# janinethoma/soft_contrastive_learning

Measured on AMD Instinct MI355X. Metric: train-step images/sec (VGG16-NetVLAD soft-MS, 640x480), higher is better.
Workload: dtype bf16; 1 GPU; configs[1]: wms soft-contrastive train step, VGG16-NetVLAD K=64, 24 images/GPU 640x480, bf16 backbone, float32-accurate NetVLAD + f32 loss; global_batch=24, locations=1200, parallelism=dp1, optimizer=adam

## Files before the change

soft_contrastive_learning_amd/csrc/convh.hip:

```cpp
#include <mutex>

#include "conv_lds.h"
#include "conv_pack_layout.h"

namespace {

constexpr int HBW = 40;
constexpr int HWC = HBW + 2;
constexpr int HPIX = 32;
constexpr int HCCH = 32;
constexpr int HNB = 128;
constexpr int HTPB = 3;
constexpr int HWT = 4 * HNB * 8;
constexpr int HTHR = 512;
constexpr int HX = 1;

template <int BHv>
struct HCfg {
  static constexpr int BH = BHv == 24 ? 12 : BHv;
  static constexpr int WR = BH + 2;
  static constexpr int SLOTS = WR * HWC * 4;
  static constexpr int NI = (SLOTS + 511) / 512;
  static constexpr int NA = (NI + 1) / 2;
  static constexpr int WIN = NI * 8 * 512;
  static constexpr int NMT = BH / 2 * 5;
  static constexpr int MT = BHv == 24 ? 15 : BH == 12 ? 8 : BH == 8 ? 10 : 4;
  static constexpr int NT = (BHv == 24 || BH == 8) ? 2 : 4;
  static constexpr int SPT = BHv == 24 ? 3 : 2;
  static constexpr int MH = MT / SPT;
  static constexpr size_t LDS = (2 * (size_t)WIN + 3 * HTPB * (size_t)HWT) * 2;
};

template <int V>
struct HConst {
  static constexpr int value = V;
};

__device__ __forceinline__ int ht_row(int i) { return (i >= 4 && i < 12) ? 1 : 0; }
__device__ __forceinline__ int ht_col(int i) { return i < 4 ? i : i < 8 ? i - 4 : i < 12 ? i - 4 : i - 8; }

__global__ __launch_bounds__(256) void convh_pack_kernel(const void* __restrict__ w, int64_t sk,
                                                         int64_t sc, int64_t sh, int64_t sw,
                                                         int flags, int cin, int kout,
                                                         unsigned short* __restrict__ packed) {
  const int transposed = flags & 1, wf32 = flags & 2;
  const int64_t idx = (int64_t)blockIdx.x * 256 + threadIdx.x;
  const int64_t total = (int64_t)9 * (cin / HCCH) * kout * HCCH;
  if (idx >= total) return;
  const int64_t off = pack_src_offset(pack_lds_coord(idx, cin), sk, sc, sh, sw, transposed);
  packed[idx] = weight_bf16(w, off, wf32);
}

template <int EPI, int BHv, bool STAMP = false, bool FULL = false>
__global__ __launch_bounds__(HTHR, 1) void convh_kernel(const unsigned short* __restrict__ x,
                                                       const unsigned short* __restrict__ packed,
                                                       int B, int H, int W, int cin, int kout,
                                                       unsigned short* __restrict__ out,
                                                       const float* __restrict__ bias, int relu,
                                                       const unsigned short* __restrict__ mask,
                                                       unsigned char* __restrict__ pidx,
                                                       int vblocks) {
  using G = HCfg<BHv>;
  constexpr int BH = G::BH, WR = G::WR, WIN = G::WIN, NMT = G::NMT, MT = G::MT, NT = G::NT;
  constexpr int MH = G::MH, NI = G::NI, NA = G::NA, SPT = G::SPT;
  constexpr bool WEAVE = BHv == 24 || BHv == 6 || BHv == 8;
  constexpr int HS = 9 * SPT;
  extern __shared__ __attribute__((aligned(16))) unsigned short lds[];
  unsigned short* win = lds;
  unsigned short* wts = lds + 2 * WIN;
  const int lane = threadIdx.x & 63;
  const int wid = __builtin_amdgcn_readfirstlane(threadIdx.x >> 6);
  const int i = lane & 15, g = lane >> 4;
  const int kb = kout / HNB;
  const int blocks_x = (W + HBW - 1) / HBW, blocks_y = (H + BH - 1) / BH;
  const int CC = cin / HCCH, S = 9 * CC;
  const unsigned short* zeros = reinterpret_cast<const unsigned short*>(zero_block);
  int nb = 0, b = 0, y0 = 0, x0 = 0;
  int rel[NI];
#pragma unroll
  for (int n = 0; n < NI; ++n) {
    const int slot = 64 * (wid + 8 * n) + lane;
    const int pix = slot >> 2, row = pix / HWC, col = pix - row * HWC;
    const int piece = (slot & 3) ^ (((col >> 2) & 1) | ((row & 1) << 1));
    rel[n] = pix >= WR * HWC ? -1 : (row << 16) | (col << 8) | piece;
  }
  int woff[NI];
  auto locate = [&](int vb) -> bool {
    const int grp = vb / (8 * kb), rem = vb - grp * 8 * kb;
    const int pblk = grp * 8 + (rem & 7);
    nb = rem >> 3;
    if (pblk >= B * blocks_x * blocks_y) return false;
    b = pblk / (blocks_x * blocks_y);
    const int t2 = pblk % (blocks_x * blocks_y);
    y0 = (t2 / blocks_x) * BH;
    x0 = (t2 % blocks_x) * HBW;
#pragma unroll
    for (int n = 0; n < NI; ++n) {
      int r = rel[n];
      asm volatile("" : "+v"(r));
      const int y = y0 - 1 + (r >> 16), xx = x0 - 1 + ((r >> 8) & 255);
      const bool inimg = r >= 0 && y >= 0 && y < H && xx >= 0 && xx < W;
      woff[n] = inimg ? ((b * H + y) * W + xx) * cin + 8 * (r & 255) : -1;
    }
    return true;
  };
  auto issue_win = [&](int cc, int buf, int n0, int n1) {
    const unsigned base = lds_byte_of(win) + buf * WIN * 2;
#pragma unroll
    for (int n = 0; n < NI; ++n)
      if (n >= n0 && n < n1)
        glds16(woff[n] >= 0 ? x + woff[n] + HCCH * cc : zeros, base + (wid + 8 * n) * 1024);
  };
  auto issue_wts = [&](int grp, int buf) {
    const unsigned short* src = packed + ((int64_t)nb * S + HTPB * grp) * HWT + lane * 8;
    const unsigned base = lds_byte_of(wts) + buf * HTPB * HWT * 2;
#pragma unroll
    for (int n = 0; n < 3; ++n) {
      const int j = wid + 8 * n;
      glds16(src + j * 512, base + j * 1024);
    }
  };
  auto issue_wts_one = [&](int grp, int buf, int n) {
    const unsigned short* src = packed + ((int64_t)nb * S + HTPB * grp) * HWT + lane * 8;
    const unsigned base = lds_byte_of(wts) + buf * HTPB * HWT * 2;
    const int j = wid + 8 * n;
    glds16(src + j * 512, base + j * 1024);
  };
  auto stage_first = [&]() {
    issue_wts(0, 0);
    issue_wts(1, 1);
    issue_win(0, 0, 0, NI);
  };
  const int mg = NT == 4 ? wid >> 1 : wid >> 2, ng = NT == 4 ? wid & 1 : wid & 3;
  constexpr bool REG = MT % 5 == 0;
  constexpr bool ALLT = NMT % MT == 0;
  int aoff[MT];
#pragma unroll
  for (int j = 0; j < MT; ++j) {
    const int mt = MT * mg + j < NMT ? MT * mg + j : NMT - 1;
    aoff[j] = ((2 * (mt / 5)) * HWC + 8 * (mt % 5)) * HPIX;
  }
  const int lane_a = (ht_row(i) * HWC + ht_col(i)) * HPIX + (REG ? 2 * (MT / 5) * mg * HWC * HPIX : 0);
  int pieces = 0;
#pragma unroll
  for (int t = 0; t < 9; ++t) {
    const int r = ht_row(i) + t / 3, c = ht_col(i) + t % 3;
    pieces |= (g ^ (((c >> 2) & 1) | ((r & 1) << 1))) << (2 * t);
  }
  const int lane_b = (g * HNB + 16 * NT * ng + i) * 8;

  const int relu_in = relu;
  const int dbg = STAMP ? 0 : SCL_DIAG_ONLY(relu >> 1);
  relu &= 1;
  const short relu_floor = relu ? (short)0 : (short)-32768;
  bool staged = false;
  if (!STAMP && (dbg & 4) && wid >= 4) __builtin_amdgcn_s_setprio(1);
  uint64_t stamp[STAMP ? 24 : 1];
  int tcount = 0;
#define HSTAMP(k)                                                                     \
  if (STAMP)                                                                          \
  asm volatile("s_memtime %0\n\ts_waitcnt lgkmcnt(0)" : "=s"(stamp[STAMP ? (k) : 0])::"memory")
  for (int vb = blockIdx.x; vb < vblocks; vb += gridDim.x) {
    HSTAMP(0);
    if (!staged) {
      if (!locate(vb)) continue;
      stage_first();
    }
    staged = false;
    const int nb_t = nb, b_t = b, y0_t = y0, x0_t = x0;

    f32x4 acc[MT][NT];
#pragma unroll
    for (int j = 0; j < MT; ++j)
#pragma unroll
      for (int n = 0; n < NT; ++n) acc[j][n] = f32x4{0.f, 0.f, 0.f, 0.f};

    u32x4 af[2][MH], bf[2][NT];
    int tb = 0;
    auto load_half = [&](const unsigned short* wbase, int h, int par, int apar) {
      const int t = h / SPT, mh = h % SPT;
      if (mh == 0) {
        const unsigned short* wbp = wts + t * HWT + lane_b;
#pragma unroll
        for (int n = 0; n < NT; ++n)
          bf[(t + par) & 1][n] = *reinterpret_cast<const u32x4*>(wbp + 16 * n * 8);
        int pk = pieces;
        asm volatile("" : "+v"(pk));
        tb = lane_a + ((pk >> (2 * t)) & 3) * 8;
      }
#pragma unroll
      for (int j = 0; j < MH; ++j)
        af[(h + apar) & 1][j] = *reinterpret_cast<const u32x4*>(
            wbase + tb +
            (REG ? (2 * ((MH * mh + j) / 5) * HWC + 8 * ((MH * mh + j) % 5)) * HPIX : aoff[MH * mh + j]) +
            ((t / 3) * HWC + t % 3) * HPIX);
    };
    const int NG = 3 * CC;
    auto chunk = [&](int cc, auto par_c) {
      constexpr int PAR = decltype(par_c)::value;
      constexpr int APAR = PAR * (HS & 1);
      const unsigned short* wcur = win + (cc & 1) * WIN;
      const unsigned short* wnext = win + ((cc + 1) & 1) * WIN;
      const int ccn = cc + 1 < CC ? cc + 1 : cc;
      auto issue_op = [&](int gi, int k) {
        if (k < 3) {
          const int gn = 3 * cc + gi + 2 < NG ? 3 * cc + gi + 2 : NG - 3 + (gi + 2) % 3;
          issue_wts_one(gn, (gi + 2) % 3, k);
        } else {
          const int n = (gi == 0 ? 0 : NA) + k - 3;
          if (gi == 0 && n < NA) issue_win(ccn, (cc + 1) & 1, n, n + 1);
          if (gi == 1 && n < NI) issue_win(ccn, (cc + 1) & 1, n, n + 1);
        }
      };
#pragma unroll
      for (int h = 0; h < HS; ++h) {
        if (h + 1 < HS)
          load_half(wcur, h + 1, PAR, APAR);
        else
          load_half(wnext, 0, PAR ^ 1, APAR ^ (HS & 1));
        __builtin_amdgcn_sched_barrier(0);
        const int t = h / SPT, mh = h % SPT;
        const bool after_barrier = WEAVE && (h % (3 * SPT) == HX + 1);
#pragma unroll
        for (int j = 0; j < MH; ++j) {
#pragma unroll
          for (int n = 0; n < NT; ++n)
            acc[MH * mh + j][n] =
                EPI == 3 ? mfma16b(af[(h + APAR) & 1][j], bf[(t + PAR) & 1][n], acc[MH * mh + j][n])
                         : mfma16b(bf[(t + PAR) & 1][n], af[(h + APAR) & 1][j], acc[MH * mh + j][n]);
          if (after_barrier) {
            __builtin_amdgcn_sched_barrier(0);
#pragma unroll
            for (int k = j * 6 / MH; k < (j + 1) * 6 / MH; ++k) issue_op(h / (3 * SPT), k);
            __builtin_amdgcn_sched_barrier(0);
          }
        }
        if (h % (3 * SPT) == HX) {
          __builtin_amdgcn_sched_barrier(0);
          const int gi = h / (3 * SPT);
          if (gi == 1)
            asm volatile("s_waitcnt vmcnt(%0)" ::"n"(NA) : "memory");
          else
            asm volatile("s_waitcnt vmcnt(0)" ::: "memory");
          HSTAMP(2 + 9 * PAR + 3 * gi);
          __builtin_amdgcn_s_barrier();
          HSTAMP(2 + 9 * PAR + 3 * gi + 1);
          if (!WEAVE) {
            const int gn = 3 * cc + gi + 2 < NG ? 3 * cc + gi + 2 : NG - 3 + (gi + 2) % 3;
            issue_wts(gn, (gi + 2) % 3);
            if (gi == 0) issue_win(ccn, (cc + 1) & 1, 0, NA);
            if (gi == 1) issue_win(ccn, (cc + 1) & 1, NA, NI);
          }
          HSTAMP(2 + 9 * PAR + 3 * gi + 2);
        }
      }
    };

    if (!(dbg & 1)) {
      asm volatile("s_waitcnt vmcnt(0)" ::: "memory");
      __syncthreads();
    }
    HSTAMP(1);
    load_half(win, 0, 0, 0);
#pragma unroll 1
    for (int cc = 0; cc < CC; cc += 2) {
      chunk(cc, HConst<0>());
      chunk(cc + 1, HConst<1>());
    }

    int nb_e = nb_t, b_e = b_t, y0_e = y0_t, x0_e = x0_t;
    asm volatile("" : "+s"(nb_e), "+s"(b_e), "+s"(y0_e), "+s"(x0_e));
    HSTAMP(20);
    __builtin_amdgcn_s_barrier();
    HSTAMP(21);
    constexpr int SLD = 16 * NT + 8;
    constexpr int PCS = 2 * NT;
    constexpr int RR = 16 * PCS / 64;
    constexpr int SCRW = 16 * SLD + 8 * (16 * NT + 16);
    static_assert(4 * SCRW <= WIN && 4 * SCRW <= HTPB * HWT, "epilogue scratch must fit");
    unsigned short* scr = wid < 4 ? lds + WIN + wid * SCRW : wts + 2 * HTPB * HWT + (wid - 4) * SCRW;
    const int ch_w = HNB * nb_e + 16 * NT * ng;
    f32x4 bias4[EPI == 1 ? NT : 1];
    float bias1[EPI == 3 ? NT : 1];
    if (EPI == 1) {
#pragma unroll
      for (int n = 0; n < NT; ++n)
        bias4[n] = *reinterpret_cast<const f32x4*>(bias + ch_w + 16 * n + 4 * g);
    }
    if (EPI == 3) {
#pragma unroll
      for (int n = 0; n < NT; ++n) bias1[n] = bias[ch_w + 16 * n + i];
    }
    int piece_o[RR], piece_px[RR];
#pragma unroll
    for (int rr = 0; rr < RR; ++rr) {
      const int pp = lane + 64 * rr;
      piece_px[rr] = pp / PCS;
      piece_o[rr] = (ht_row(pp / PCS) * W + ht_col(pp / PCS)) * kout + 8 * (pp % PCS);
    }
    constexpr int PD = MT / 2;
    u32x4 mk[EPI == 2 ? MT : 1][EPI == 2 ? RR : 1];
    const int64_t tile_off = (((int64_t)b_e * H + y0_e) * W + x0_e) * kout + ch_w;
    const bool full_tile = FULL ? !(dbg & 2) : (y0_e + BH <= H && x0_e + HBW <= W && !(dbg & 2));
    auto load_mask = [&](int j) {
      const int mt = MT * mg + j;
      const int oy = y0_e + 2 * (mt / 5), ox = x0_e + 8 * (mt % 5);
      const unsigned short* mb = mask + tile_off + ((2 * (mt / 5)) * W + 8 * (mt % 5)) * kout;
#pragma unroll
      for (int rr = 0; rr < RR; ++rr) {
        if (FULL ? (ALLT || mt < NMT) : (full_tile && mt < NMT)) {
          mk[EPI == 2 ? j : 0][EPI == 2 ? rr : 0] = *reinterpret_cast<const u32x4*>(mb + piece_o[rr]);
        } else if (FULL) {
          mk[EPI == 2 ? j : 0][EPI == 2 ? rr : 0] = u32x4{0u, 0u, 0u, 0u};
        } else {
          const bool inside = mt < NMT && oy + ht_row(piece_px[rr]) < H && ox + ht_col(piece_px[rr]) < W;
          mk[EPI == 2 ? j : 0][EPI == 2 ? rr : 0] =
              inside ? *reinterpret_cast<const u32x4*>(mb + piece_o[rr]) : u32x4{0u, 0u, 0u, 0u};
        }
      }
    };
    if (EPI == 2) {
#pragma unroll
      for (int j = 0; j < PD; ++j) load_mask(j);
    }

    auto stage_next = [&]() {
      const int vn = vb + gridDim.x;
      if (vn < vblocks && locate(vn)) {
        asm volatile("s_waitcnt vmcnt(0)" ::: "memory");
        stage_first();
        staged = true;
      }
    };
    if (EPI != 2) stage_next();

    if (EPI == 3) {
      const int PH = H / 2, PW = W / 2;
      const bool upper = g == 0 || g == 3;
      const int cb = g < 2 ? 0 : 4;
      unsigned char* scr8 = reinterpret_cast<unsigned char*>(scr + 16 * SLD);
      constexpr int SLD8 = 16 * NT + 16;
#pragma unroll
      for (int jb = 0; jb < MT; jb += 4) {
#pragma unroll
        for (int jj = 0; jj < 4; ++jj) {
          const int j = jb + jj < MT ? jb + jj : MT - 1;
#pragma unroll
          for (int n = 0; n < NT; ++n) {
#pragma unroll
            for (int q0 = 0; q0 < 4; q0 += 2) {
              const float v0 = acc[j][n][q0], v1 = acc[j][n][q0 + 1];
              const float lm = fmaxf(v0, v1);
              const int li = v0 >= v1 ? 0 : 1;
              const float om = __shfl_xor(lm, 16);
              const int oi = __shfl_xor(li, 16);
              const float mu = upper ? lm : om, ml = upper ? om : lm;
              const int iu = upper ? li : oi, il = upper ? oi : li;
              const float m = fmaxf(mu, ml);
              const int k = mu >= ml ? iu : 2 + il;
              const int pl = 4 * jj + ((cb + q0) >> 1);
              if (upper) {
                scr[pl * SLD + 16 * n + i] = f32_to_bf16(fmaxf(m + bias1[n], 0.f));
                scr8[pl * SLD8 + 16 * n + i] = (unsigned char)k;
              }
            }
          }
        }
        __builtin_amdgcn_wave_barrier();
#pragma unroll
        for (int rr = 0; rr < RR; ++rr) {
          const int pp = lane + 64 * rr, pl = pp / PCS, pc = pp % PCS;
          const int mt = MT * mg + jb + (pl >> 2);
          const int py = (y0_e >> 1) + mt / 5, px = (x0_e >> 1) + 4 * (mt % 5) + (pl & 3);
          const u32x4 v = *reinterpret_cast<const u32x4*>(scr + pl * SLD + 8 * pc);
          if (jb + (pl >> 2) < MT && (FULL ? (ALLT || mt < NMT) : (mt < NMT && py < PH && px < PW && !(dbg & 2))))
            *reinterpret_cast<u32x4*>(out + (((int64_t)b_e * PH + py) * PW + px) * kout + ch_w + 8 * pc) = v;
        }
        if (lane < 16 * NT) {
          const int pl = lane / NT, pc = lane % NT;
          const int mt = MT * mg + jb + (pl >> 2);
          const int py = (y0_e >> 1) + mt / 5, px = (x0_e >> 1) + 4 * (mt % 5) + (pl & 3);
          const u32x4 v = *reinterpret_cast<const u32x4*>(scr8 + pl * SLD8 + 16 * pc);
          if (jb + (pl >> 2) < MT && (FULL ? (ALLT || mt < NMT) : (mt < NMT && py < PH && px < PW && !(dbg & 2))))
            *reinterpret_cast<u32x4*>(pidx + (((int64_t)b_e * PH + py) * PW + px) * kout + ch_w + 16 * pc) = v;
        }
        __builtin_amdgcn_wave_barrier();
      }
    } else {
      unsigned short* out_tile = out + tile_off;
#pragma unroll
      for (int j = 0; j < MT; ++j) {
        const int mt = MT * mg + j;
        if (ALLT || mt < NMT) {
          const int oy = y0_e + 2 * (mt / 5), ox = x0_e + 8 * (mt % 5);
          unsigned short* ob = out_tile + ((2 * (mt / 5)) * W + 8 * (mt % 5)) * kout;
#pragma unroll
          for (int n = 0; n < NT; ++n) {
            f32x4 v = acc[j][n];
            if (EPI == 1) v += bias4[n];
            unsigned p0 = pack2_bf16(v[0], v[1]), p1 = pack2_bf16(v[2], v[3]);
            if (EPI == 1) {
              p0 = max2_i16(p0, relu_floor);
              p1 = max2_i16(p1, relu_floor);
            }
            const u32x2 pk = {p0, p1};
            *reinterpret_cast<u32x2*>(scr + i * SLD + 16 * n + 4 * g) = pk;
          }
          __builtin_amdgcn_wave_barrier();
#pragma unroll
          for (int rr = 0; rr < RR; ++rr) {
            u32x4 v = *reinterpret_cast<const u32x4*>(scr + piece_px[rr] * SLD + 8 * ((lane + 64 * rr) % PCS));
            if (EPI == 2) v = relu_mask(v, mk[EPI == 2 ? j : 0][EPI == 2 ? rr : 0]);
            if (full_tile) {
              *reinterpret_cast<u32x4*>(ob + piece_o[rr]) = v;
            } else if (!FULL) {
              const bool inside = oy + ht_row(piece_px[rr]) < H && ox + ht_col(piece_px[rr]) < W && !(dbg & 2);
              if (inside) *reinterpret_cast<u32x4*>(ob + piece_o[rr]) = v;
            }
          }
          __builtin_amdgcn_wave_barrier();
        }
        if (EPI == 2) {
          __builtin_amdgcn_sched_barrier(0);
          if (j + PD < MT) load_mask(j + PD);
          if (j + PD == MT - 1) stage_next();
          __builtin_amdgcn_sched_barrier(0);
        }
      }
    }
    if (STAMP) {
      HSTAMP(22);
      if (threadIdx.x == 64 * ((relu_in >> 4) & 7) && (tcount == 1 || tcount == 2)) {
        uint64_t* o = reinterpret_cast<uint64_t*>(out + (int64_t)B * H * W * kout) +
                      (int64_t)(blockIdx.x * 2 + tcount - 1) * 24;
#pragma unroll
        for (int k = 0; k < 23; ++k) o[k] = stamp[STAMP ? k : 0];
      }
      ++tcount;
    }
  }
#undef HSTAMP
}

}

struct HGeom {
  const unsigned short* packed;
  int bh;
  LdsConvGrid grid;
};

template <int E, int BHV, bool STAMP = false, bool FULL = false>
static void convh_run(const LdsConvCall& c, const HGeom& g, int relu) {
  if constexpr (!STAMP && !FULL)
    if (c.H % HCfg<BHV>::BH == 0 && c.W % HBW == 0) return convh_run<E, BHV, false, true>(c, g, relu);
  static SclDeviceOnce once;
  scl_call_once(once, [] {
    (void)hipFuncSetAttribute(reinterpret_cast<const void*>(&convh_kernel<E, BHV, STAMP, FULL>),
                              hipFuncAttributeMaxDynamicSharedMemorySize, (int)HCfg<BHV>::LDS);
  });
  SCL_LAUNCH("convh_kernel", (convh_kernel<E, BHV, STAMP, FULL>), dim3(g.grid.gsize), dim3(HTHR),
             HCfg<BHV>::LDS, c.stream, (const unsigned short*)c.x, g.packed, c.B, c.H, c.W, c.cin,
             c.kout, (unsigned short*)c.out, c.bias, relu, (const unsigned short*)c.mask,
             (unsigned char*)c.pidx, g.grid.vblocks);
}
template <int BHV>
static void convh_epilogue(const LdsConvCall& c, const HGeom& g, int dbgbits) {
  if (c.pidx) convh_run<3, BHV>(c, g, dbgbits);
  else if (c.mask) convh_run<2, BHV>(c, g, dbgbits);
  else if (c.bias) convh_run<1, BHV>(c, g, (c.relu ? 1 : 0) | dbgbits);
  else convh_run<0, BHV>(c, g, 0);
}

#ifdef SCL_DIAG
static bool convh_diag(const LdsConvCall& c, const HGeom& g, int* rc);
#endif

int convh_launch(const LdsConvCall& c) {
  const int dv = SCL_DIAG_ONLY(c.dv);
  HGeom g;
  g.packed = (const unsigned short*)c.workspace;
  if (c.flags & SCL_W_PACKED) {
    g.packed = (const unsigned short*)c.w;
  } else {
    const int64_t total = (int64_t)9 * (c.cin / HCCH) * c.kout * HCCH;
    SCL_LAUNCH("convh_pack_kernel", convh_pack_kernel, dim3((unsigned)((total + 255) / 256)),
               dim3(256), 0, c.stream, c.w, c.sk, c.sc, c.sh, c.sw, c.flags, c.cin, c.kout,
               (unsigned short*)c.workspace);
  }
  const int bx = (c.W + HBW - 1) / HBW, kb = c.kout / HNB;
  const int cus = scl_conv_cus();
  g.bh = 12;
  int64_t best = -1;
  for (int cand : {12, 8, 6}) {
    const int64_t wg = (int64_t)c.B * ((c.H + cand - 1) / cand) * bx * kb;
    const int64_t cost = ((wg + cus - 1) / cus) * (cand + 2);
    if (best < 0 || cost < best) {
      best = cost;
      g.bh = cand;
    }
  }
  if (dv == 3012 || dv == 3008 || dv == 3006) g.bh = dv - 3000;
  if (dv == 3013) g.bh = 12;
  g.grid = lds_conv_grid((int64_t)c.B * ((c.H + g.bh - 1) / g.bh) * bx, kb, cus, dv);
#ifdef SCL_DIAG
  {
    int rc;
    if (convh_diag(c, g, &rc)) return rc;
  }
#endif
  const int dbgbits = (dv >= 3020 && dv < 3024) ? (dv - 3020) << 1 : (dv == 3040 ? 4 << 1 : 0);
  if (g.bh == 12) convh_epilogue<24>(c, g, dbgbits);
  else if (g.bh == 8) convh_epilogue<8>(c, g, dbgbits);
  else convh_epilogue<6>(c, g, dbgbits);
  return scl_launch_status();
}
```

soft_contrastive_learning_amd/csrc/convh_diag.hip:

```cpp
#include "convh.hip"

static bool convh_diag(const LdsConvCall& c, const HGeom& g, int* rc) {
  const int dv = c.dv;
  const bool stamps = dv >= 3024 && dv < 3040 && c.bias && !c.mask && !c.pidx && g.bh == 12;
  if (dv != 3012 && !stamps) return false;
  if (dv == 3012)
    convh_epilogue<12>(c, g, 0);
  else if (dv < 3032)
    convh_run<1, 24, true>(c, g, (c.relu ? 1 : 0) | ((dv - 3024) << 4));
  else
    convh_run<1, 12, true>(c, g, (c.relu ? 1 : 0) | ((dv - 3032) << 4));
  *rc = scl_launch_status();
  return true;
}
```

Measured before the change: 2054 images/sec.

## Prefetch next tile's input window and weights during last K-chunk of conv

In the persistent 3x3 conv kernel, the next tile's input window and first weight groups are now prefetched while the final channel chunks of the current tile are still computing, wrapping the weight-group index and window chunk around. Previously the kernel drained the pipeline and staged the next tile synchronously in the epilogue. This removes the per-tile pipeline bubble between tiles. In exchange the tile locate logic and the index arithmetic get more complex, the epilogue lane indexing is hidden from the compiler, and the old path is kept behind a diagnostic flag.

```diff
diff --git a/soft_contrastive_learning_amd/csrc/convh.hip b/soft_contrastive_learning_amd/csrc/convh.hip
--- a/soft_contrastive_learning_amd/csrc/convh.hip
+++ b/soft_contrastive_learning_amd/csrc/convh.hip
@@ -85,15 +85,16 @@
     rel[n] = pix >= WR * HWC ? -1 : (row << 16) | (col << 8) | piece;
   }
   int woff[NI];
-  auto locate = [&](int vb) -> bool {
+  auto locate = [&](int vb, bool offsets = true) -> bool {
     const int grp = vb / (8 * kb), rem = vb - grp * 8 * kb;
     const int pblk = grp * 8 + (rem & 7);
     nb = rem >> 3;
-    if (pblk >= B * blocks_x * blocks_y) return false;
     b = pblk / (blocks_x * blocks_y);
     const int t2 = pblk % (blocks_x * blocks_y);
     y0 = (t2 / blocks_x) * BH;
     x0 = (t2 % blocks_x) * HBW;
+    if (pblk >= B * blocks_x * blocks_y) return false;
+    if (!offsets) return true;
 #pragma unroll
     for (int n = 0; n < NI; ++n) {
       int r = rel[n];
@@ -150,7 +151,8 @@
   const int lane_b = (g * HNB + 16 * NT * ng + i) * 8;
 
   const int relu_in = relu;
-  const int dbg = STAMP ? 0 : SCL_DIAG_ONLY(relu >> 1);
+  const int dbg = STAMP ? 0 : SCL_DIAG_ONLY((relu >> 1) & 7);
+  const bool oldb = SCL_DIAG_ONLY(((relu >> (STAMP ? 7 : 4)) & 1) != 0);
   relu &= 1;
   const short relu_floor = relu ? (short)0 : (short)-32768;
   bool staged = false;
@@ -165,6 +167,8 @@
     if (!staged) {
       if (!locate(vb)) continue;
       stage_first();
+    } else {
+      locate(vb, false);
     }
     staged = false;
     const int nb_t = nb, b_t = b, y0_t = y0, x0_t = x0;
@@ -196,16 +200,20 @@
             ((t / 3) * HWC + t % 3) * HPIX);
     };
     const int NG = 3 * CC;
+    bool pref = false;
     auto chunk = [&](int cc, auto par_c) {
       constexpr int PAR = decltype(par_c)::value;
       constexpr int APAR = PAR * (HS & 1);
       const unsigned short* wcur = win + (cc & 1) * WIN;
       const unsigned short* wnext = win + ((cc + 1) & 1) * WIN;
-      const int ccn = cc + 1 < CC ? cc + 1 : cc;
+      const int ccn = cc + 1 < CC ? cc + 1 : pref ? 0 : cc;
+      auto next_group = [&](int gi) {
+        const int gw = 3 * cc + gi + 2;
+        return gw < NG ? gw : oldb ? NG - 3 + (gi + 2) % 3 : gw - NG;
+      };
       auto issue_op = [&](int gi, int k) {
         if (k < 3) {
-          const int gn = 3 * cc + gi + 2 < NG ? 3 * cc + gi + 2 : NG - 3 + (gi + 2) % 3;
-          issue_wts_one(gn, (gi + 2) % 3, k);
+          issue_wts_one(next_group(gi), (gi + 2) % 3, k);
         } else {
           const int n = (gi == 0 ? 0 : NA) + k - 3;
           if (gi == 0 && n < NA) issue_win(ccn, (cc + 1) & 1, n, n + 1);
@@ -246,8 +254,7 @@
           __builtin_amdgcn_s_barrier();
           HSTAMP(2 + 9 * PAR + 3 * gi + 1);
           if (!WEAVE) {
-            const int gn = 3 * cc + gi + 2 < NG ? 3 * cc + gi + 2 : NG - 3 + (gi + 2) % 3;
-            issue_wts(gn, (gi + 2) % 3);
+            issue_wts(next_group(gi), (gi + 2) % 3);
             if (gi == 0) issue_win(ccn, (cc + 1) & 1, 0, NA);
             if (gi == 1) issue_win(ccn, (cc + 1) & 1, NA, NI);
           }
@@ -265,8 +272,13 @@
 #pragma unroll 1
     for (int cc = 0; cc < CC; cc += 2) {
       chunk(cc, HConst<0>());
+      if (cc + 2 >= CC && !oldb) {
+        const int vn = vb + gridDim.x;
+        if (vn < vblocks && locate(vn)) pref = true;
+      }
       chunk(cc + 1, HConst<1>());
     }
+    staged = pref;
 
     int nb_e = nb_t, b_e = b_t, y0_e = y0_t, x0_e = x0_t;
     asm volatile("" : "+s"(nb_e), "+s"(b_e), "+s"(y0_e), "+s"(x0_e));
@@ -326,7 +338,7 @@
 
     auto stage_next = [&]() {
       const int vn = vb + gridDim.x;
-      if (vn < vblocks && locate(vn)) {
+      if (oldb && vn < vblocks && locate(vn)) {
         asm volatile("s_waitcnt vmcnt(0)" ::: "memory");
         stage_first();
         staged = true;
@@ -336,8 +348,11 @@
 
     if (EPI == 3) {
       const int PH = H / 2, PW = W / 2;
-      const bool upper = g == 0 || g == 3;
-      const int cb = g < 2 ? 0 : 4;
+      int le = lane;
+      asm volatile("" : "+v"(le));
+      const int ie = le & 15, ge = le >> 4;
+      const bool upper = ge == 0 || ge == 3;
+      const int cb = ge < 2 ? 0 : 4;
       unsigned char* scr8 = reinterpret_cast<unsigned char*>(scr + 16 * SLD);
       constexpr int SLD8 = 16 * NT + 16;
 #pragma unroll
@@ -360,8 +375,8 @@
               const int k = mu >= ml ? iu : 2 + il;
               const int pl = 4 * jj + ((cb + q0) >> 1);
               if (upper) {
-                scr[pl * SLD + 16 * n + i] = f32_to_bf16(fmaxf(m + bias1[n], 0.f));
-                scr8[pl * SLD8 + 16 * n + i] = (unsigned char)k;
+                scr[pl * SLD + 16 * n + ie] = f32_to_bf16(fmaxf(m + bias1[n], 0.f));
+                scr8[pl * SLD8 + 16 * n + ie] = (unsigned char)k;
               }
             }
           }
@@ -369,15 +384,15 @@
         __builtin_amdgcn_wave_barrier();
 #pragma unroll
         for (int rr = 0; rr < RR; ++rr) {
-          const int pp = lane + 64 * rr, pl = pp / PCS, pc = pp % PCS;
+          const int pp = le + 64 * rr, pl = pp / PCS, pc = pp % PCS;
           const int mt = MT * mg + jb + (pl >> 2);
           const int py = (y0_e >> 1) + mt / 5, px = (x0_e >> 1) + 4 * (mt % 5) + (pl & 3);
           const u32x4 v = *reinterpret_cast<const u32x4*>(scr + pl * SLD + 8 * pc);
           if (jb + (pl >> 2) < MT && (FULL ? (ALLT || mt < NMT) : (mt < NMT && py < PH && px < PW && !(dbg & 2))))
             *reinterpret_cast<u32x4*>(out + (((int64_t)b_e * PH + py) * PW + px) * kout + ch_w + 8 * pc) = v;
         }
-        if (lane < 16 * NT) {
-          const int pl = lane / NT, pc = lane % NT;
+        if (le < 16 * NT) {
+          const int pl = le / NT, pc = le % NT;
           const int mt = MT * mg + jb + (pl >> 2);
           const int py = (y0_e >> 1) + mt / 5, px = (x0_e >> 1) + 4 * (mt % 5) + (pl & 3);
           const u32x4 v = *reinterpret_cast<const u32x4*>(scr8 + pl * SLD8 + 16 * pc);
@@ -469,7 +484,7 @@
   if (c.pidx) convh_run<3, BHV>(c, g, dbgbits);
   else if (c.mask) convh_run<2, BHV>(c, g, dbgbits);
   else if (c.bias) convh_run<1, BHV>(c, g, (c.relu ? 1 : 0) | dbgbits);
-  else convh_run<0, BHV>(c, g, 0);
+  else convh_run<0, BHV>(c, g, dbgbits & 16);
 }
 
 #ifdef SCL_DIAG
@@ -509,7 +524,7 @@
     if (convh_diag(c, g, &rc)) return rc;
   }
 #endif
-  const int dbgbits = (dv >= 3020 && dv < 3024) ? (dv - 3020) << 1 : (dv == 3040 ? 4 << 1 : 0);
+  const int dbgbits = (dv >= 3020 && dv < 3024) ? (dv - 3020) << 1 : dv == 3040 ? 4 << 1 : dv == 3041 ? 16 : 0;
   if (g.bh == 12) convh_epilogue<24>(c, g, dbgbits);
   else if (g.bh == 8) convh_epilogue<8>(c, g, dbgbits);
   else convh_epilogue<6>(c, g, dbgbits);
diff --git a/soft_contrastive_learning_amd/csrc/convh_diag.hip b/soft_contrastive_learning_amd/csrc/convh_diag.hip
--- a/soft_contrastive_learning_amd/csrc/convh_diag.hip
+++ b/soft_contrastive_learning_amd/csrc/convh_diag.hip
@@ -2,12 +2,14 @@
 
 static bool convh_diag(const LdsConvCall& c, const HGeom& g, int* rc) {
   const int dv = c.dv;
-  const bool stamps = dv >= 3024 && dv < 3040 && c.bias && !c.mask && !c.pidx && g.bh == 12;
+  const bool stamps = ((dv >= 3024 && dv < 3040) || (dv >= 3042 && dv < 3050)) && c.bias && !c.mask && !c.pidx && g.bh == 12;
   if (dv != 3012 && !stamps) return false;
   if (dv == 3012)
     convh_epilogue<12>(c, g, 0);
   else if (dv < 3032)
     convh_run<1, 24, true>(c, g, (c.relu ? 1 : 0) | ((dv - 3024) << 4));
+  else if (dv >= 3042)
+    convh_run<1, 24, true>(c, g, (c.relu ? 1 : 0) | ((dv - 3042) << 4) | 128);
   else
     convh_run<1, 12, true>(c, g, (c.relu ? 1 : 0) | ((dv - 3032) << 4));
   *rc = scl_launch_status();
```

After: 2053 images/sec, median of 3. No clear change (-0.0%).
